# 123-code/Distributed-neural-networks

Measured on AMD Instinct MI355X. Metric: images/sec CIFAR-10 2-stage, higher is better.
Workload: dtype fp32 (bf16x3 split emulation, ~2^-16 per product); 1 GPU; model=cifar10-convnet (cifar_model_parts.py NeuralNetwork), global_batch=65536, parallelism=pp2-colocated, stages=2, microbatches=1, stage0_spare_cus=0, p2p=none, stage_cut=conv|fc (reference split, 16 KiB/img hop)

## Files before the change

### csrc/kernels/cifar_x3.hip

```cpp
#include <type_traits>

#include "gemm_epilogue.h"

namespace dnn {
namespace x3 {

template <bool PK>
__device__ __forceinline__ void split2(float a, float b, uint32_t& hi, uint32_t& lo) {
  if constexpr (PK) {
    hi = pack2bf_pk(a, b);
    const float ah = __uint_as_float(hi << 16), bh = __uint_as_float(hi & 0xffff0000u);
    float da = a - ah;
    const float db = b - bh;
    asm("" : "+v"(da));
    lo = pack2bf_pk(da, db);
  } else {
    hi = pack2bf(a, b);
    const float ah = __uint_as_float(hi << 16), bh = __uint_as_float(hi & 0xffff0000u);
    lo = pack2bf(a - ah, b - bh);
  }
}

__device__ __forceinline__ float4 buf_load16(const void* base, int bytes, int voff, int soff) {
#if defined(__HIP_DEVICE_COMPILE__)
  const auto rsrc = __builtin_amdgcn_make_buffer_rsrc(const_cast<void*>(base), 0, bytes, 0x00020000);
  return __builtin_bit_cast(float4, __builtin_amdgcn_raw_buffer_load_b128(rsrc, voff, soff, 0));
#else
  return float4{};
#endif
}
__device__ __forceinline__ void buf_glds16(const void* base, int bytes, int voff, int soff, void* lds_wave_base) {
#if defined(__HIP_DEVICE_COMPILE__)
  const auto rsrc = __builtin_amdgcn_make_buffer_rsrc(const_cast<void*>(base), 0, bytes, 0x00020000);
  __builtin_amdgcn_raw_ptr_buffer_load_lds(rsrc, (LDS_AS void*)lds_wave_base, 16, voff, soff, 0, 0);
#endif
}

__device__ __forceinline__ int dpp_xor1(int v) { return __builtin_amdgcn_mov_dpp(v, 0xB1, 0xF, 0xF, false); }
__device__ __forceinline__ int dpp_xor2(int v) { return __builtin_amdgcn_mov_dpp(v, 0x4E, 0xF, 0xF, false); }

constexpr int XW = 40;
constexpr int XPL = 34 * XW * 8;
constexpr int A1PL = 18 * 18 * 64;
constexpr int XP32 = 224;
constexpr int XPL32 = 34 * XP32;

template <int C1>
__device__ __forceinline__ constexpr int xpl() {
  return C1 ? XPL32 : XPL;
}
template <int C1>
__device__ __forceinline__ constexpr int lds_bytes() {
  return 4 * xpl<C1>() + 4 * A1PL;
}
constexpr int TAB_BYTES = 3 * 256 * 4;
struct U8Input {
  const unsigned char* x;
  const uint32_t* table;
};
template <int IN>
using s0_input_t = std::conditional_t<IN == 1, U8Input, const float* __restrict__>;

template <int C1>
__device__ __forceinline__ int xin_off(int k, int lo) {
  return ((k & 1) * 2 + lo) * xpl<C1>();
}
template <int C1>
__device__ __forceinline__ int a1_off(int k, int lo) {
  return 4 * xpl<C1>() + ((k & 1) * 2 + lo) * A1PL;
}

template <int S, int I, int LO>
__device__ __forceinline__ constexpr int c2_imm() {
  return (8 * I + (S >> 1) % 3) * 64 + LO * A1PL;
}

template <int S>
__device__ __forceinline__ void c2_issue(const uint32_t (&b)[3][2], bf16x8 (&a)[4]) {
  constexpr int ky = (S >> 1) / 3, par = S & 1;
  asm volatile("ds_read_b128 %0, %1 offset:%2" : "=v"(a[0]) : "v"(b[ky][par]), "i"(c2_imm<S, 0, 0>()));
  asm volatile("ds_read_b128 %0, %1 offset:%2" : "=v"(a[1]) : "v"(b[ky][par]), "i"(c2_imm<S, 1, 0>()));
  asm volatile("ds_read_b128 %0, %1 offset:%2" : "=v"(a[2]) : "v"(b[ky][par]), "i"(c2_imm<S, 0, 1>()));
  asm volatile("ds_read_b128 %0, %1 offset:%2" : "=v"(a[3]) : "v"(b[ky][par]), "i"(c2_imm<S, 1, 1>()));
}

template <int S>
__device__ __forceinline__ void c2_step(const uint32_t (&b)[3][2], const bf16x8 (&wh)[18], const bf16x8 (&wl)[18],
                                        f32x16 (&acc)[2], bf16x8 (&cur)[4], bf16x8 (&nxt)[4]) {
  if constexpr (S + 1 < 18) {
    c2_issue<S + 1>(b, nxt);
    asm volatile("s_waitcnt lgkmcnt(4)" ::: "memory");
  } else {
    asm volatile("s_waitcnt lgkmcnt(0)" ::: "memory");
  }
  __builtin_amdgcn_sched_barrier(0);
  acc[0] = __builtin_amdgcn_mfma_f32_32x32x16_bf16(cur[0], wh[S], acc[0], 0, 0, 0);
  acc[1] = __builtin_amdgcn_mfma_f32_32x32x16_bf16(cur[1], wh[S], acc[1], 0, 0, 0);
  acc[0] = __builtin_amdgcn_mfma_f32_32x32x16_bf16(cur[0], wl[S], acc[0], 0, 0, 0);
  acc[1] = __builtin_amdgcn_mfma_f32_32x32x16_bf16(cur[1], wl[S], acc[1], 0, 0, 0);
  acc[0] = __builtin_amdgcn_mfma_f32_32x32x16_bf16(cur[2], wh[S], acc[0], 0, 0, 0);
  acc[1] = __builtin_amdgcn_mfma_f32_32x32x16_bf16(cur[3], wh[S], acc[1], 0, 0, 0);
  __builtin_amdgcn_sched_barrier(0);
  if constexpr (S + 1 < 18) c2_step<S + 1>(b, wh, wl, acc, nxt, cur);
}

template <int N>
__device__ __forceinline__ void resident_fence(const bf16x8 (&w)[N]) {
#pragma unroll
  for (int i = 0; i < N; ++i) asm volatile("" ::"v"(w[i]));
}

template <int C2>
__device__ __forceinline__ int a1_swz(int Y) {
  return C2 ? (2 * Y) & 3 : Y & 3;
}

template <int T, int J, int LO>
__device__ __forceinline__ constexpr int m16_imm() {
  return (((T >> 1) / 3) * 18 + 4 * (2 * (T & 1) + J) + (T >> 1) % 3) * 64 + LO * A1PL;
}

template <int T>
__device__ __forceinline__ void m16_issue(const uint32_t (&b)[2], bf16x8 (&a)[4]) {
  constexpr int kyp = ((T >> 1) / 3) & 1;
  asm volatile("ds_read_b128 %0, %1 offset:%2" : "=v"(a[0]) : "v"(b[kyp]), "i"(m16_imm<T, 0, 0>()));
  asm volatile("ds_read_b128 %0, %1 offset:%2" : "=v"(a[1]) : "v"(b[kyp]), "i"(m16_imm<T, 1, 0>()));
  asm volatile("ds_read_b128 %0, %1 offset:%2" : "=v"(a[2]) : "v"(b[kyp]), "i"(m16_imm<T, 0, 1>()));
  asm volatile("ds_read_b128 %0, %1 offset:%2" : "=v"(a[3]) : "v"(b[kyp]), "i"(m16_imm<T, 1, 1>()));
}

template <int T>
__device__ __forceinline__ void m16_step(const uint32_t (&b)[2], const bf16x8 (&wh)[2][9], const bf16x8 (&wl)[2][9],
                                         f32x4 (&acc)[4][2], bf16x8 (&cur)[4], bf16x8 (&nxt)[4]) {
  constexpr int tap = T >> 1, m0 = 2 * (T & 1);
  if constexpr (T + 1 < 18) {
    m16_issue<T + 1>(b, nxt);
    asm volatile("s_waitcnt lgkmcnt(4)" ::: "memory");
  } else {
    asm volatile("s_waitcnt lgkmcnt(0)" ::: "memory");
  }
  __builtin_amdgcn_sched_barrier(0);
#pragma unroll
  for (int term = 0; term < 3; ++term)
#pragma unroll
    for (int nt = 0; nt < 2; ++nt)
#pragma unroll
      for (int j = 0; j < 2; ++j)
        acc[m0 + j][nt] = __builtin_amdgcn_mfma_f32_16x16x32_bf16(cur[(term == 2 ? 2 : 0) + j],
                                                                  term == 1 ? wl[nt][tap] : wh[nt][tap], acc[m0 + j][nt], 0, 0, 0);
  __builtin_amdgcn_sched_barrier(0);
  if constexpr (T + 1 < 18) m16_step<T + 1>(b, wh, wl, acc, nxt, cur);
}

template <bool SPLIT_OUT, int NT>
__device__ __forceinline__ void m16_epilogue(const f32x4 (&acc)[4][2], float bias, float* img, int oc, int PY, int x1) {
  float v[4];
#pragma unroll
  for (int mt = 0; mt < 4; ++mt) {
    const f32x4& a = acc[mt][NT];
    v[mt] = fmaxf(fmax_nan(fmax_nan(a[0], a[1]), fmax_nan(a[2], a[3])) + bias, 0.f);
  }
  const auto s0 = __builtin_amdgcn_permlane16_swap(__float_as_uint(v[0]), __float_as_uint(v[2]), false, false);
  const auto s1 = __builtin_amdgcn_permlane16_swap(__float_as_uint(v[1]), __float_as_uint(v[3]), false, false);
  if constexpr (SPLIT_OUT) {
    uint2 hi, lo;
    split2<true>(__uint_as_float(s0[0]), __uint_as_float(s0[1]), hi.x, lo.x);
    split2<true>(__uint_as_float(s1[0]), __uint_as_float(s1[1]), hi.y, lo.y);
    char* bp = reinterpret_cast<char*>(img) + (oc * 2 + (PY >> 2)) * 128 + ((PY & 3) * 8 + 4 * x1) * 2;
    *reinterpret_cast<uint2*>(bp) = hi;
    *reinterpret_cast<uint2*>(bp + 64) = lo;
  } else {
    *reinterpret_cast<uint4*>(img + oc * 64 + PY * 8 + 4 * x1) = make_uint4(s0[0], s0[1], s1[0], s1[1]);
  }
}

}

using namespace x3;

template <bool WIDE, bool SPLIT_OUT, int C2 = 0, int C1 = 0, int IN = 0>
__global__ __launch_bounds__(512, 1) void cifar_stage0_x3_kernel(
    s0_input_t<IN> x, float* __restrict__ out, const bf16_t* __restrict__ w1h,
    const bf16_t* __restrict__ w1l, const float* __restrict__ b1, const bf16_t* __restrict__ w2h,
    const bf16_t* __restrict__ w2l, const float* __restrict__ b2, int B) {
  static_assert(IN == 0 || C1 == 1, "uint8 input exists in the K = 32 producer only");
  constexpr int LDS_BYTES = lds_bytes<C1>();
  __shared__ __attribute__((aligned(16))) char smem[LDS_BYTES + (IN ? TAB_BYTES : 0)];
  const int tid = threadIdx.x, lane = tid & 63;
  const int wave = __builtin_amdgcn_readfirstlane(tid >> 6);
  const bool producer = wave < 4;
  const int rw = wave & 3;
  const int rt = tid & 255;
  const int h = lane >> 5, r32 = lane & 31;
  const int n = B > (int)blockIdx.x ? (B - 1 - (int)blockIdx.x) / (int)gridDim.x + 1 : 0;

  for (int i = tid; i < LDS_BYTES / 16; i += 512) reinterpret_cast<uint4*>(smem)[i] = make_uint4(0, 0, 0, 0);
  if constexpr (IN == 1)
    for (int i = tid; i < TAB_BYTES / 4; i += 512) reinterpret_cast<uint32_t*>(smem + LDS_BYTES)[i] = x.table[i];

  __syncthreads();

  if (producer) {
    const float bias = b1[r32];
    asm volatile("" ::"v"(bias));
    const int q = ((r32 & 1) ? 2 : 0) + ((r32 & 2) ? 1 : 0);
    const int cb = r32 & ~3;

    auto conv1_store = [&](const float (&v)[4], int Y0, int X0, int k) {
      const bool odd = r32 & 1;
      const int s0 = __float_as_int(odd ? v[0] : v[2]), s1 = __float_as_int(odd ? v[1] : v[3]);
      const float r0 = __int_as_float(dpp_xor1(s0)), r1 = __int_as_float(dpp_xor1(s1));
      uint32_t u0h, u0l, u1h, u1l;
      if (!odd) {
        split2<true>(v[0], r0, u0h, u0l);
        split2<true>(v[1], r1, u1h, u1l);
      } else {
        split2<true>(r0, v[2], u0h, u0l);
        split2<true>(r1, v[3], u1h, u1l);
      }
      const bool hi2 = r32 & 2;
      const uint32_t rch = (uint32_t)dpp_xor2((int)(hi2 ? u0h : u1h));
      const uint32_t rcl = (uint32_t)dpp_xor2((int)(hi2 ? u0l : u1l));
      const uint32_t mh = hi2 ? u1h : u0h, ml = hi2 ? u1l : u0l;
      uint2 wh, wl;
      wh.x = hi2 ? rch : mh;
      wh.y = hi2 ? mh : rch;
      wl.x = hi2 ? rcl : ml;
      wl.y = hi2 ? ml : rcl;
      const int Y = Y0 + (q >> 1), X = X0 + (q & 1);
      const int o = (Y * 18 + X) * 64 + ((((cb >> 3) ^ a1_swz<C2>(Y))) << 4) + (cb & 7) * 2;
      *reinterpret_cast<uint2*>(smem + a1_off<C1>(k, 0) + o) = wh;
      *reinterpret_cast<uint2*>(smem + a1_off<C1>(k, 1) + o) = wl;
    };
    auto produce = [&](auto&& load_img, auto&& stage_img, auto&& conv1_img) {
      if (n > 0) {
        load_img(0);
        stage_img(0);
        if (n > 1) load_img(1);
      }
      __syncthreads();
      for (int it = 0; it <= n; ++it) {
        if (it < n) {
          conv1_img(it);
          if (it + 1 < n) {
            stage_img(it + 1);
            if (it + 2 < n) load_img(it + 2);
          }
        }
        __syncthreads();
      }
    };

    if constexpr (C1 == 0 && IN == 0) {
      bf16x8 w1hf[3], w1lf[3];
#pragma unroll
      for (int s = 0; s < 3; ++s) {
        w1hf[s] = *reinterpret_cast<const bf16x8*>(w1h + r32 * 48 + s * 16 + h * 8);
        w1lf[s] = *reinterpret_cast<const bf16x8*>(w1l + r32 * 48 + s * 16 + h * 8);
      }
      resident_fence(w1hf);
      resident_fence(w1lf);

      float pf[4][3];
      auto load_img = [&](int k) {
        const float* xb = x + (size_t)(blockIdx.x + (size_t)k * gridDim.x) * 3072;
#pragma unroll
        for (int i = 0; i < 4; ++i)
#pragma unroll
          for (int c = 0; c < 3; ++c) pf[i][c] = xb[c * 1024 + rt + 256 * i];
      };
      auto stage_img = [&](int k) {
        char* xh = smem + xin_off<C1>(k, 0);
        char* xl = smem + xin_off<C1>(k, 1);
#pragma unroll
        for (int i = 0; i < 4; ++i) {
          const int p = rt + 256 * i, yy = p >> 5, xx = p & 31;
          uint2 vh, vl;
          split2<true>(pf[i][0], pf[i][1], vh.x, vl.x);
          split2<true>(pf[i][2], 0.f, vh.y, vl.y);
          const int o = ((yy + 1) * XW + xx + 1) * 8;
          *reinterpret_cast<uint2*>(xh + o) = vh;
          *reinterpret_cast<uint2*>(xl + o) = vl;
        }
      };
      const int c1_lane = ((r32 >> 3) * XW + (r32 & 7) + 2 * h) * 8;

      auto conv1_epi = [&](int t, const f32x16& acc, int k) {
        const int ty = t >> 2, tx = t & 3;
        float v[4];
#pragma unroll
        for (int qy = 0; qy < 2; ++qy)
#pragma unroll
          for (int qx = 0; qx < 2; ++qx) {
            const int g0 = (2 * qy) * 4 + 2 * qx;
            v[qy * 2 + qx] =
                fmaxf(fmax_nan(fmax_nan(acc[g0], acc[g0 + 1]), fmax_nan(acc[g0 + 4], acc[g0 + 5])) + bias, 0.f);
          }
        conv1_store(v, 2 * ty + 1, 4 * tx + 2 * h + 1, k);
      };
      auto frag = [&](const char* p) {
        const uint2 a = *reinterpret_cast<const uint2*>(p);
        const uint2 b = *reinterpret_cast<const uint2*>(p + 8);
        return __builtin_bit_cast(bf16x8, make_uint4(a.x, a.y, b.x, b.y));
      };
      auto conv1_pair = [&](int ta, int tb, int k) {
        const char* xh = smem + xin_off<C1>(k, 0);
        const int oa = c1_lane + ((4 * (ta >> 2)) * XW + 8 * (ta & 3)) * 8;
        const int ob = c1_lane + ((4 * (tb >> 2)) * XW + 8 * (tb & 3)) * 8;
        bf16x8 fah[3], fal[3], fbh[3], fbl[3];
#pragma unroll
        for (int s = 0; s < 3; ++s) {
          fah[s] = frag(xh + oa + s * XW * 8);
          fbh[s] = frag(xh + ob + s * XW * 8);
          fal[s] = frag(xh + XPL + oa + s * XW * 8);
          fbl[s] = frag(xh + XPL + ob + s * XW * 8);
        }
        f32x16 acca = {}, accb = {};
#pragma unroll
        for (int s = 0; s < 3; ++s) {
          acca = __builtin_amdgcn_mfma_f32_32x32x16_bf16(fah[s], w1hf[s], acca, 0, 0, 0);
          accb = __builtin_amdgcn_mfma_f32_32x32x16_bf16(fbh[s], w1hf[s], accb, 0, 0, 0);
          acca = __builtin_amdgcn_mfma_f32_32x32x16_bf16(fah[s], w1lf[s], acca, 0, 0, 0);
          accb = __builtin_amdgcn_mfma_f32_32x32x16_bf16(fbh[s], w1lf[s], accb, 0, 0, 0);
          acca = __builtin_amdgcn_mfma_f32_32x32x16_bf16(fal[s], w1hf[s], acca, 0, 0, 0);
          accb = __builtin_amdgcn_mfma_f32_32x32x16_bf16(fbl[s], w1hf[s], accb, 0, 0, 0);
        }
        conv1_epi(ta, acca, k);
        conv1_epi(tb, accb, k);
      };
      produce(load_img, stage_img, [&](int it) {
#pragma unroll 1
        for (int t = rw; t < 32; t += 8) conv1_pair(t, t + 4, it);
      });
    } else if constexpr (C1 == 1) {
      bf16x8 w1hf[2][2], w1lf[2][2];
#pragma unroll
      for (int par = 0; par < 2; ++par)
#pragma unroll
        for (int s = 0; s < 2; ++s) {
          w1hf[par][s] = *reinterpret_cast<const bf16x8*>(w1h + par * 1024 + r32 * 32 + s * 16 + h * 8);
          w1lf[par][s] = *reinterpret_cast<const bf16x8*>(w1l + par * 1024 + r32 * 32 + s * 16 + h * 8);
        }
      resident_fence(w1hf[0]);
      resident_fence(w1hf[1]);
      resident_fence(w1lf[0]);
      resident_fence(w1lf[1]);

      const int sj = rt & 7, r5 = rt >> 3;
      const int sy = (r5 & ~3) | ((r5 & 1) << 1) | ((r5 >> 1) & 1);
      std::conditional_t<IN == 1, uint32_t, float4> pf[3];
      auto load_img = [&](int k) {
        if constexpr (IN == 1) {
          const unsigned char* xb = x.x + (size_t)(blockIdx.x + (size_t)k * gridDim.x) * 3072 + sy * 96 + sj * 12;
#pragma unroll
          for (int c = 0; c < 3; ++c) pf[c] = *reinterpret_cast<const uint32_t*>(xb + 4 * c);
        } else {
          const float* xb = x + (size_t)(blockIdx.x + (size_t)k * gridDim.x) * 3072 + sy * 32 + sj * 4;
#pragma unroll
          for (int c = 0; c < 3; ++c) pf[c] = *reinterpret_cast<const float4*>(xb + c * 1024);
        }
      };
      auto stage_img = [&](int k) {
        const int o = (sy + 1) * XP32 + 8 + 24 * sj;
        char* xh = smem + xin_off<C1>(k, 0) + o;
        char* xl = smem + xin_off<C1>(k, 1) + o;
        uint2 vh[3], vl[3];
        if constexpr (IN == 1) {
          const char* tab = smem + LDS_BYTES;
          uint32_t e[12];
#pragma unroll
          for (int i = 0; i < 12; ++i)
            e[i] = *reinterpret_cast<const uint32_t*>(tab + (i % 3) * 1024 + ((pf[i >> 2] >> (8 * (i & 3))) & 0xffu) * 4);
          uint32_t ph[6], pl[6];
#pragma unroll
          for (int i = 0; i < 6; ++i) {
            ph[i] = __builtin_amdgcn_perm(e[2 * i + 1], e[2 * i], 0x05040100u);
            pl[i] = __builtin_amdgcn_perm(e[2 * i + 1], e[2 * i], 0x07060302u);
          }
#pragma unroll
          for (int i = 0; i < 3; ++i) {
            vh[i] = make_uint2(ph[2 * i], ph[2 * i + 1]);
            vl[i] = make_uint2(pl[2 * i], pl[2 * i + 1]);
          }
        } else {
          split2<true>(pf[0].x, pf[1].x, vh[0].x, vl[0].x);
          split2<true>(pf[2].x, pf[0].y, vh[0].y, vl[0].y);
          split2<true>(pf[1].y, pf[2].y, vh[1].x, vl[1].x);
          split2<true>(pf[0].z, pf[1].z, vh[1].y, vl[1].y);
          split2<true>(pf[2].z, pf[0].w, vh[2].x, vl[2].x);
          split2<true>(pf[1].w, pf[2].w, vh[2].y, vl[2].y);
        }
#pragma unroll
        for (int i = 0; i < 3; ++i) {
          *reinterpret_cast<uint2*>(xh + 8 * i) = vh[i];
          *reinterpret_cast<uint2*>(xl + 8 * i) = vl[i];
        }
      };
      const int rr = r32 >> 3, cc = r32 & 7;
      const int l0 = (rr + 2 * h) * XP32 + 12 * cc;
      int l1[4];
#pragma unroll
      for (int i = 0; i < 4; ++i)
        l1[i] = h ? (rr + (i < 2 ? i : 2)) * XP32 + 12 * cc + 16 : (rr + 1) * XP32 + 12 * cc + 4 * i;
      auto ld32 = [&](const char* p) { return *reinterpret_cast<const uint32_t*>(p); };
      auto conv1_pair = [&](int tp, int k) {
        const int ty = tp >> 1, tx2 = tp & 1;
        const char* xh = smem + xin_off<C1>(k, 0) + 4 * ty * XP32 + 96 * tx2;
        bf16x8 f[2][2][2];
#pragma unroll
        for (int par = 0; par < 2; ++par)
#pragma unroll
          for (int pl = 0; pl < 2; ++pl) {
            const char* p = xh + pl * XPL32 + 8 * par;
            f[par][pl][0] = __builtin_bit_cast(
                bf16x8, make_uint4(ld32(p + l0), ld32(p + l0 + 4), ld32(p + l0 + 8), ld32(p + l0 + 12)));
            f[par][pl][1] = __builtin_bit_cast(
                bf16x8, make_uint4(ld32(p + l1[0]), ld32(p + l1[1]), ld32(p + l1[2]), ld32(p + l1[3])));
          }
        f32x16 acca = {}, accb = {};
#pragma unroll
        for (int s = 0; s < 2; ++s) {
          acca = __builtin_amdgcn_mfma_f32_32x32x16_bf16(f[0][0][s], w1hf[0][s], acca, 0, 0, 0);
          accb = __builtin_amdgcn_mfma_f32_32x32x16_bf16(f[1][0][s], w1hf[1][s], accb, 0, 0, 0);
          acca = __builtin_amdgcn_mfma_f32_32x32x16_bf16(f[0][0][s], w1lf[0][s], acca, 0, 0, 0);
          accb = __builtin_amdgcn_mfma_f32_32x32x16_bf16(f[1][0][s], w1lf[1][s], accb, 0, 0, 0);
          acca = __builtin_amdgcn_mfma_f32_32x32x16_bf16(f[0][1][s], w1hf[0][s], acca, 0, 0, 0);
          accb = __builtin_amdgcn_mfma_f32_32x32x16_bf16(f[1][1][s], w1hf[1][s], accb, 0, 0, 0);
        }
#pragma unroll
        for (int e = 0; e < 2; ++e) {
          float v[4];
#pragma unroll
          for (int qy = 0; qy < 2; ++qy)
#pragma unroll
            for (int qx = 0; qx < 2; ++qx) {
              const int g = 8 * qy + 2 * e + qx;
              v[qy * 2 + qx] =
                  fmaxf(fmax_nan(fmax_nan(acca[g], accb[g]), fmax_nan(acca[g + 4], accb[g + 4])) + bias, 0.f);
            }
          conv1_store(v, 2 * ty + 1, 8 * tx2 + 4 * h + 2 * e + 1, k);
        }
      };
      produce(load_img, stage_img, [&](int it) {
#pragma unroll 1
        for (int tp = rw; tp < 16; tp += 4) conv1_pair(tp, it);
      });
    }
  } else if constexpr (C2 != 0) {
    const int m = lane & 15, q16 = lane >> 4, y1 = q16 >> 1, x1 = q16 & 1;
    const int oc = (rw & 1) * 32 + m;
    bf16x8 w2hf[2][9], w2lf[2][9];
#pragma unroll
    for (int nt = 0; nt < 2; ++nt)
#pragma unroll
      for (int tap = 0; tap < 9; ++tap) {
        w2hf[nt][tap] = *reinterpret_cast<const bf16x8*>(w2h + (oc + 16 * nt) * 288 + tap * 32 + q16 * 8);
        w2lf[nt][tap] = *reinterpret_cast<const bf16x8*>(w2l + (oc + 16 * nt) * 288 + tap * 32 + q16 * 8);
      }
    const float bias0 = b2[oc], bias1 = b2[oc + 16];
    resident_fence(w2hf[0]);
    resident_fence(w2hf[1]);
    resident_fence(w2lf[0]);
    resident_fence(w2lf[1]);
    asm volatile("" ::"v"(bias0), "v"(bias1));
    const int py = 2 * (m >> 3) + ((m >> 1) & 1), px = 2 * ((m >> 2) & 1) + (m & 1);
    uint32_t lb[2];
#pragma unroll
    for (int kyp = 0; kyp < 2; ++kyp) lb[kyp] = (uint32_t)((py * 18 + px) * 64 + ((q16 ^ a1_swz<C2>(py + kyp)) << 4));

    auto conv2_img = [&](int k) {
      float* img = out + (size_t)(blockIdx.x + (size_t)k * gridDim.x) * 4096;
      const uint32_t plane = (uint32_t)(uintptr_t)(smem + a1_off<C1>(k, 0));
#pragma unroll 1
      for (int p = 0; p < 2; ++p) {
        const int ty2 = (rw >> 1) * 2 + p;
        const uint32_t rb = plane + ty2 * 4 * 18 * 64;
        const uint32_t b[2] = {rb + lb[0], rb + lb[1]};
        f32x4 acc[4][2];
#pragma unroll
        for (int mt = 0; mt < 4; ++mt) acc[mt][0] = acc[mt][1] = f32x4{};
        bf16x8 a0[4], a1[4];
        m16_issue<0>(b, a0);
        m16_step<0>(b, w2hf, w2lf, acc, a0, a1);
        m16_epilogue<SPLIT_OUT, 0>(acc, bias0, img, oc, 2 * ty2 + y1, x1);
        m16_epilogue<SPLIT_OUT, 1>(acc, bias1, img, oc + 16, 2 * ty2 + y1, x1);
      }
    };

    __syncthreads();
    for (int it = 0; it <= n; ++it) {
      if (it >= 1) conv2_img(it - 1);
      __syncthreads();
    }
  } else {
    const int oc2 = (rw & 1) * 32 + r32;
    bf16x8 w2hf[18], w2lf[18];
#pragma unroll
    for (int s = 0; s < 18; ++s) {
      w2hf[s] = *reinterpret_cast<const bf16x8*>(w2h + oc2 * 288 + s * 16 + h * 8);
      w2lf[s] = *reinterpret_cast<const bf16x8*>(w2l + oc2 * 288 + s * 16 + h * 8);
    }
    const float bias = b2[oc2];
    resident_fence(w2hf);
    resident_fence(w2lf);
    asm volatile("" ::"v"(bias));
    uint32_t lb[3][2];
#pragma unroll
    for (int ky = 0; ky < 3; ++ky)
#pragma unroll
      for (int par = 0; par < 2; ++par) {
        const int yr = (r32 >> 3) + ky;
        lb[ky][par] = (uint32_t)((yr * 18 + (r32 & 7)) * 64 + (((2 * par + h) ^ (yr & 3)) << 4));
      }

    auto conv2_img = [&](int k) {
      float* ob = out + (size_t)(blockIdx.x + (size_t)k * gridDim.x) * 4096 + oc2 * 64;
      const uint32_t plane = (uint32_t)(uintptr_t)(smem + a1_off<C1>(k, 0));
#pragma unroll 1
      for (int p = 0; p < 2; ++p) {
        const int ty2 = (rw >> 1) * 2 + p;
        const uint32_t rb = plane + ty2 * 4 * 18 * 64;
        uint32_t b[3][2];
#pragma unroll
        for (int ky = 0; ky < 3; ++ky)
#pragma unroll
          for (int par = 0; par < 2; ++par) b[ky][par] = rb + lb[ky][par];
        f32x16 acc[2] = {f32x16{}, f32x16{}};
        bf16x8 a0[4], a1[4];
        c2_issue<0>(b, a0);
        c2_step<0>(b, w2hf, w2lf, acc, a0, a1);
        if constexpr (WIDE) {
#pragma unroll
          for (int qy = 0; qy < 2; ++qy) {
            const int g0 = (2 * qy) * 4;
            float v[2][2];
#pragma unroll
            for (int i = 0; i < 2; ++i) {
              v[i][0] = fmaxf(fmax_nan(fmax_nan(acc[i][g0], acc[i][g0 + 1]), fmax_nan(acc[i][g0 + 4], acc[i][g0 + 5])) + bias, 0.f);
              v[i][1] = fmaxf(fmax_nan(fmax_nan(acc[i][g0 + 2], acc[i][g0 + 3]), fmax_nan(acc[i][g0 + 6], acc[i][g0 + 7])) + bias,
                              0.f);
            }
            const auto sx = __builtin_amdgcn_permlane32_swap(__float_as_uint(v[0][0]), __float_as_uint(v[1][0]), false,
                                                             false);
            const auto sy = __builtin_amdgcn_permlane32_swap(__float_as_uint(v[0][1]), __float_as_uint(v[1][1]), false,
                                                             false);
            const int PY = 2 * ty2 + qy;
            if constexpr (SPLIT_OUT) {
              uint2 hi, lo;
              split2<true>(__uint_as_float(sx[0]), __uint_as_float(sy[0]), hi.x, lo.x);
              split2<true>(__uint_as_float(sx[1]), __uint_as_float(sy[1]), hi.y, lo.y);
              char* bp = reinterpret_cast<char*>(ob - oc2 * 64) + (oc2 * 2 + (PY >> 2)) * 128 + ((PY & 3) * 8 + 4 * h) * 2;
              *reinterpret_cast<uint2*>(bp) = hi;
              *reinterpret_cast<uint2*>(bp + 64) = lo;
            } else {
              *reinterpret_cast<uint4*>(ob + PY * 8 + 4 * h) = make_uint4(sx[0], sy[0], sx[1], sy[1]);
            }
          }
        } else {
#pragma unroll
        for (int i = 0; i < 2; ++i) {
#pragma unroll
          for (int qy = 0; qy < 2; ++qy) {
            float2 pv;
            const int g0 = (2 * qy) * 4;
            pv.x = fmaxf(fmax_nan(fmax_nan(acc[i][g0], acc[i][g0 + 1]), fmax_nan(acc[i][g0 + 4], acc[i][g0 + 5])) + bias, 0.f);
            pv.y = fmaxf(fmax_nan(fmax_nan(acc[i][g0 + 2], acc[i][g0 + 3]), fmax_nan(acc[i][g0 + 6], acc[i][g0 + 7])) + bias,
                         0.f);
            const int PY = 2 * ty2 + qy, PX = 4 * i + 2 * h;
            if constexpr (SPLIT_OUT) {
              uint32_t hi, lo;
              split2<true>(pv.x, pv.y, hi, lo);
              char* bp = reinterpret_cast<char*>(ob - oc2 * 64) + (oc2 * 2 + (PY >> 2)) * 128 + ((PY & 3) * 8 + PX) * 2;
              *reinterpret_cast<uint32_t*>(bp) = hi;
              *reinterpret_cast<uint32_t*>(bp + 64) = lo;
            } else {
              *reinterpret_cast<float2*>(ob + PY * 8 + PX) = pv;
            }
          }
        }
        }
      }
    };

    __syncthreads();
    for (int it = 0; it <= n; ++it) {
      if (it >= 1) conv2_img(it - 1);
      __syncthreads();
    }
  }
}

constexpr int F1_T = 256, F1_K = 32, F1_PLANE = 256 * 64;

__device__ __forceinline__ int f1_swz(int r) { return (r >> 2) & 2; }

__device__ __forceinline__ bf16x8 f1_frag(const char* plane, int row, int chunk) {
  return *reinterpret_cast<const bf16x8*>(plane + row * 64 + ((chunk ^ f1_swz(row)) << 4));
}

__device__ __forceinline__ void f1_tile_coords(int logical, int ntm, int ntn, int& tm, int& tn) {
  constexpr int G = 8;
  const int per = G * ntn, grp = logical / per, first = grp * G;
  const int gm = min(ntm - first, G), r = logical - grp * per;
  tm = first + r % gm;
  tn = r / gm;
}

template <bool SPLIT_IN, bool LEAN>
__global__ __launch_bounds__(512, 1) void cifar_fc1_x3_kernel(const float* __restrict__ A, int lda,
                                                              const bf16_t* __restrict__ Wh,
                                                              const bf16_t* __restrict__ Wl, int ldw,
                                                              const float* __restrict__ bias, float* __restrict__ C,
                                                              int ldc, int M, int N, int K) {
  __shared__ __attribute__((aligned(1024))) char smem[2 * 4 * F1_PLANE];
  const int tid = threadIdx.x, lane = tid & 63, wave = tid >> 6;
  const int ntn = N / F1_T, ntm = (M + F1_T - 1) / F1_T;
  int tm, tn;
  f1_tile_coords(xcd_remap(blockIdx.x, ntm * ntn), ntm, ntn, tm, tn);
  const int m0 = tm * F1_T, n0 = tn * F1_T;
  const int wr = wave >> 2, wc = wave & 3;
  const int nk = K / F1_K;
  auto plane = [&](int u, int p) { return smem + (u * 4 + p) * F1_PLANE; };

  int ltid = tid;
  float4 ar[4];
  const int wave_u = __builtin_amdgcn_readfirstlane(wave);
  int a_rows[4];
#pragma unroll
  for (int k = 0; k < 4; ++k) a_rows[k] = __builtin_amdgcn_readfirstlane(max(min(M - m0 - 64 * k, 64), 0));
  const float* const a_tile = A + (size_t)m0 * lda;
  const int a_tile_bytes = min(M - m0, F1_T) * lda * 4;
  auto dma_voff = [&](int ld_bytes) {
    return (wave * 32 + (lane >> 2)) * ld_bytes + (((lane & 3) ^ ((lane >> 4) & 2)) << 4);
  };
  int a_voff = 0, a_voff1 = 0, w_voff = 0;
  LDS_AS char* aw_base = nullptr;
  LDS_AS char* fa_base = nullptr;
  LDS_AS char* fw_base = nullptr;
  if constexpr (LEAN) {
    LDS_AS char* const lds = (LDS_AS char*)smem;
    const int fr = lane & 15, fc = lane >> 4;
    const int fo = fr * 64 + ((fc ^ ((fr >> 2) & 2)) << 4);
    fa_base = lds + (wave >> 2) * 128 * 64 + fo;
    fw_base = lds + 2 * F1_PLANE + (wave & 3) * 64 * 64 + fo;
    w_voff = dma_voff(ldw * 2);
    if constexpr (SPLIT_IN) {
      a_voff = dma_voff(lda * 4);
      a_voff1 = a_voff + 16 * lda * 4;
      asm volatile("" : "+v"(a_voff1));
    } else {
      const int r = tid >> 3, c = (tid & 7) >> 1, half = tid & 1;
      a_voff = r * lda * 4 + (tid & 7) * 16;
      aw_base = lds + r * 64 + ((c ^ f1_swz(r)) << 4) + half * 8;
      asm volatile("" : "+v"(aw_base));
    }
    asm volatile("" : "+v"(a_voff), "+v"(w_voff), "+v"(fa_base), "+v"(fw_base));
  }
  constexpr int F1_BUF = 4 * F1_PLANE;
  auto load_a = [&](int t, auto) {
    if constexpr (LEAN) {
#pragma unroll
      for (int k = 0; k < 4; ++k)
        ar[k] = buf_load16(A + (size_t)(m0 + 64 * k) * lda, a_rows[k] * lda * 4, a_voff, t * 128);
      return;
    }
    const int x = ltid;
#pragma unroll
    for (int k = 0; k < 4; ++k) {
      const int row = min(m0 + (x >> 3) + 64 * k, M - 1);
      ar[k] = *reinterpret_cast<const float4*>(A + (size_t)row * lda + t * F1_K + (x & 7) * 4);
    }
  };
  auto store_a = [&](int u, auto) {
    if constexpr (LEAN) {
      LDS_AS char* const w = aw_base + u * F1_BUF;
#pragma unroll
      for (int k = 0; k < 4; ++k) {
        uint2 hi, lo;
        split2<true>(ar[k].x, ar[k].y, hi.x, lo.x);
        split2<true>(ar[k].z, ar[k].w, hi.y, lo.y);
        typedef uint32_t u32x2 __attribute__((ext_vector_type(2)));
        *reinterpret_cast<LDS_AS u32x2*>(w + k * 4096) = u32x2{hi.x, hi.y};
        *reinterpret_cast<LDS_AS u32x2*>(w + F1_PLANE + k * 4096) = u32x2{lo.x, lo.y};
      }
      return;
    }
    const int x = ltid;
#pragma unroll
    for (int k = 0; k < 4; ++k) {
      const int r = (x >> 3) + 64 * k, c = (x & 7) >> 1, half = x & 1;
      uint2 hi, lo;
      split2<false>(ar[k].x, ar[k].y, hi.x, lo.x);
      split2<false>(ar[k].z, ar[k].w, hi.y, lo.y);
      const int o = r * 64 + ((c ^ f1_swz(r)) << 4) + half * 8;
      *reinterpret_cast<uint2*>(plane(u, 0) + o) = hi;
      *reinterpret_cast<uint2*>(plane(u, 1) + o) = lo;
    }
  };
  auto stage_a = [&](int u, int t) {
    if constexpr (LEAN) {
#pragma unroll
      for (int p = 0; p < 2; ++p)
#pragma unroll
        for (int j = 0; j < 2; ++j)
          buf_glds16(a_tile, a_tile_bytes, j ? a_voff1 : a_voff, t * 128 + p * 64,
                     plane(u, p) + (wave_u * 2 + j) * 1024);
      return;
    }
    const char* Ab = reinterpret_cast<const char*>(A);
    const int lane = ltid & 63, wave = ltid >> 6;
#pragma unroll
    for (int p = 0; p < 2; ++p) {
#pragma unroll
      for (int j = 0; j < 2; ++j) {
        const int piece = wave * 2 + j, rl = piece * 16 + (lane >> 2);
        const int c = (lane & 3) ^ f1_swz(rl);
        const int row = min(m0 + rl, M - 1);
        glds16(Ab + (size_t)row * lda * 4 + t * 128 + p * 64 + c * 16, plane(u, p) + piece * 1024);
      }
    }
  };
  auto stage_w = [&](int u, int t) {
    if constexpr (LEAN) {
#pragma unroll
      for (int p = 0; p < 2; ++p)
#pragma unroll
        for (int j = 0; j < 2; ++j)
          buf_glds16((p ? Wl : Wh) + (size_t)n0 * ldw, F1_T * ldw * 2, w_voff, j * 16 * ldw * 2 + t * 64,
                     plane(u, 2 + p) + (wave_u * 2 + j) * 1024);
      return;
    }
    const int lane = ltid & 63, wave = ltid >> 6;
#pragma unroll
    for (int p = 0; p < 2; ++p) {
      const bf16_t* W = p ? Wl : Wh;
#pragma unroll
      for (int j = 0; j < 2; ++j) {
        const int piece = wave * 2 + j, rl = piece * 16 + (lane >> 2);
        const int c = (lane & 3) ^ f1_swz(rl);
        glds16(W + (size_t)(n0 + rl) * ldw + t * F1_K + c * 8, plane(u, 2 + p) + piece * 1024);
      }
    }
  };

  f32x4 acc[8][4];
#pragma unroll
  for (int i = 0; i < 8; ++i)
#pragma unroll
    for (int j = 0; j < 4; ++j) acc[i][j] = f32x4{0.f, 0.f, 0.f, 0.f};

  using I0 = std::integral_constant<int, 0>;
  if constexpr (SPLIT_IN) {
    stage_a(0, 0);
    stage_w(0, 0);
    asm volatile("s_waitcnt vmcnt(0)" ::: "memory");
  } else {
    load_a(0, I0{});
    stage_w(0, 0);
    asm volatile("s_waitcnt vmcnt(0)" ::: "memory");
    store_a(0, I0{});
    if (nk > 1) load_a(1, I0{});
  }
  asm volatile("s_waitcnt lgkmcnt(0)" ::: "memory");
  __builtin_amdgcn_sched_barrier(0);
  __builtin_amdgcn_s_barrier();
  __builtin_amdgcn_sched_barrier(0);

  const int fr = lane & 15, fc = lane >> 4;
  auto barrier = [&]() {
    asm volatile("s_waitcnt lgkmcnt(0)" ::: "memory");
    __builtin_amdgcn_sched_barrier(0);
    __builtin_amdgcn_s_barrier();
    __builtin_amdgcn_sched_barrier(0);
  };
  bf16x8 fbh[4], fbl[4], fah[8], fal[8];
  auto read_frags = [&](int u) {
    if constexpr (LEAN) {
      LDS_AS char* const fw = fw_base + u * F1_BUF;
      LDS_AS char* const fa = fa_base + u * F1_BUF;
#pragma unroll
      for (int j = 0; j < 4; ++j) {
        fbh[j] = *reinterpret_cast<LDS_AS bf16x8*>(fw + j * 1024);
        fbl[j] = *reinterpret_cast<LDS_AS bf16x8*>(fw + F1_PLANE + j * 1024);
      }
#pragma unroll
      for (int i = 0; i < 8; ++i) {
        fah[i] = *reinterpret_cast<LDS_AS bf16x8*>(fa + i * 1024);
        fal[i] = *reinterpret_cast<LDS_AS bf16x8*>(fa + F1_PLANE + i * 1024);
      }
      return;
    }
    const int fr = ltid & 15, fc = (ltid >> 4) & 3, wc = (ltid >> 6) & 3, wr = ltid >> 8;
#pragma unroll
    for (int j = 0; j < 4; ++j) {
      fbh[j] = f1_frag(plane(u, 2), wc * 64 + j * 16 + fr, fc);
      fbl[j] = f1_frag(plane(u, 3), wc * 64 + j * 16 + fr, fc);
    }
#pragma unroll
    for (int i = 0; i < 8; ++i) {
      fah[i] = f1_frag(plane(u, 0), wr * 128 + i * 16 + fr, fc);
      fal[i] = f1_frag(plane(u, 1), wr * 128 + i * 16 + fr, fc);
    }
  };
  auto mfma_seg = [&]() {
    __builtin_amdgcn_sched_barrier(0);
#pragma unroll
    for (int i = 0; i < 8; ++i)
#pragma unroll
      for (int term = 0; term < 3; ++term)
#pragma unroll
        for (int j = 0; j < 4; ++j)
          acc[i][j] = __builtin_amdgcn_mfma_f32_16x16x32_bf16(term == 1 ? fbl[j] : fbh[j], term == 2 ? fal[i] : fah[i],
                                                              acc[i][j], 0, 0, 0);
    __builtin_amdgcn_sched_barrier(0);
  };
  auto retire_dma = [&](bool a_in_flight) {
    if (a_in_flight)
      asm volatile("s_waitcnt vmcnt(4)" ::: "memory");
    else
      asm volatile("s_waitcnt vmcnt(0)" ::: "memory");
  };
  auto stage_next = [&](int u, int t) {
    if constexpr (SPLIT_IN) stage_a(u, t);
    stage_w(u, t);
  };
  const bool g1 = __builtin_amdgcn_readfirstlane(wr) != 0;
  auto fresh_tid = [&]() {
    if constexpr (LEAN) return;
    ltid = tid;
    asm volatile("" : "+v"(ltid));
  };
// ... 348 lines not shown
```

Baseline: 31.84 million images/s.

## Raise conv2 wave priority early and use buffer loads/stores with precomputed lane offsets

```diff
diff --git a/csrc/kernels/cifar_x3.hip b/csrc/kernels/cifar_x3.hip
--- a/csrc/kernels/cifar_x3.hip
+++ b/csrc/kernels/cifar_x3.hip
@@ -29,6 +29,28 @@
   return float4{};
 #endif
 }
+__device__ __forceinline__ uint32_t buf_load4(const void* base, int bytes, int voff, int soff) {
+#if defined(__HIP_DEVICE_COMPILE__)
+  const auto rsrc = __builtin_amdgcn_make_buffer_rsrc(const_cast<void*>(base), 0, bytes, 0x00020000);
+  return __builtin_amdgcn_raw_buffer_load_b32(rsrc, voff, soff, 0);
+#else
+  return 0;
+#endif
+}
+__device__ __forceinline__ void buf_store16(void* base, int bytes, int voff, int soff, uint4 v) {
+#if defined(__HIP_DEVICE_COMPILE__)
+  typedef unsigned int u32x4 __attribute__((ext_vector_type(4)));
+  const auto rsrc = __builtin_amdgcn_make_buffer_rsrc(base, 0, bytes, 0x00020000);
+  __builtin_amdgcn_raw_buffer_store_b128(u32x4{v.x, v.y, v.z, v.w}, rsrc, voff, soff, 0);
+#endif
+}
+__device__ __forceinline__ void buf_store8(void* base, int bytes, int voff, int soff, uint2 v) {
+#if defined(__HIP_DEVICE_COMPILE__)
+  typedef unsigned int u32x2 __attribute__((ext_vector_type(2)));
+  const auto rsrc = __builtin_amdgcn_make_buffer_rsrc(base, 0, bytes, 0x00020000);
+  __builtin_amdgcn_raw_buffer_store_b64(u32x2{v.x, v.y}, rsrc, voff, soff, 0);
+#endif
+}
 __device__ __forceinline__ void buf_glds16(const void* base, int bytes, int voff, int soff, void* lds_wave_base) {
 #if defined(__HIP_DEVICE_COMPILE__)
   const auto rsrc = __builtin_amdgcn_make_buffer_rsrc(const_cast<void*>(base), 0, bytes, 0x00020000);
@@ -44,6 +66,7 @@
 constexpr int A1PL = 18 * 18 * 64;
 constexpr int XP32 = 224;
 constexpr int XPL32 = 34 * XP32;
+constexpr int C2_PRIO_STEPS = 9;
 
 template <int C1>
 __device__ __forceinline__ constexpr int xpl() {
@@ -87,6 +110,7 @@
 template <int S>
 __device__ __forceinline__ void c2_step(const uint32_t (&b)[3][2], const bf16x8 (&wh)[18], const bf16x8 (&wl)[18],
                                         f32x16 (&acc)[2], bf16x8 (&cur)[4], bf16x8 (&nxt)[4]) {
+  if constexpr (S == C2_PRIO_STEPS) __builtin_amdgcn_s_setprio(0);
   if constexpr (S + 1 < 18) {
     c2_issue<S + 1>(b, nxt);
     asm volatile("s_waitcnt lgkmcnt(4)" ::: "memory");
@@ -133,6 +157,7 @@
 __device__ __forceinline__ void m16_step(const uint32_t (&b)[2], const bf16x8 (&wh)[2][9], const bf16x8 (&wl)[2][9],
                                          f32x4 (&acc)[4][2], bf16x8 (&cur)[4], bf16x8 (&nxt)[4]) {
   constexpr int tap = T >> 1, m0 = 2 * (T & 1);
+  if constexpr (T == C2_PRIO_STEPS) __builtin_amdgcn_s_setprio(0);
   if constexpr (T + 1 < 18) {
     m16_issue<T + 1>(b, nxt);
     asm volatile("s_waitcnt lgkmcnt(4)" ::: "memory");
@@ -153,7 +178,7 @@
 }
 
 template <bool SPLIT_OUT, int NT>
-__device__ __forceinline__ void m16_epilogue(const f32x4 (&acc)[4][2], float bias, float* img, int oc, int PY, int x1) {
+__device__ __forceinline__ void m16_epilogue(const f32x4 (&acc)[4][2], float bias, float* img, int lane, int p) {
   float v[4];
 #pragma unroll
   for (int mt = 0; mt < 4; ++mt) {
@@ -166,11 +191,10 @@
     uint2 hi, lo;
     split2<true>(__uint_as_float(s0[0]), __uint_as_float(s0[1]), hi.x, lo.x);
     split2<true>(__uint_as_float(s1[0]), __uint_as_float(s1[1]), hi.y, lo.y);
-    char* bp = reinterpret_cast<char*>(img) + (oc * 2 + (PY >> 2)) * 128 + ((PY & 3) * 8 + 4 * x1) * 2;
-    *reinterpret_cast<uint2*>(bp) = hi;
-    *reinterpret_cast<uint2*>(bp + 64) = lo;
+    buf_store8(img, 16384, lane, 32 * p + 4096 * NT, hi);
+    buf_store8(img, 16384, lane, 32 * p + 4096 * NT + 64, lo);
   } else {
-    *reinterpret_cast<uint4*>(img + oc * 64 + PY * 8 + 4 * x1) = make_uint4(s0[0], s0[1], s1[0], s1[1]);
+    buf_store16(img, 16384, lane, 64 * p + 4096 * NT, make_uint4(s0[0], s0[1], s1[0], s1[1]));
   }
 }
 
@@ -206,18 +230,18 @@
     const int q = ((r32 & 1) ? 2 : 0) + ((r32 & 2) ? 1 : 0);
     const int cb = r32 & ~3;
 
-    auto conv1_store = [&](const float (&v)[4], int Y0, int X0, int k) {
+    auto a1_lane = [&](int par, int xh) {
+      const int Y = 2 * par + 1 + (q >> 1);
+      return ((q >> 1) * 18 + (q & 1) + xh) * 64 + ((((cb >> 3) ^ a1_swz<C2>(Y))) << 4) + (cb & 7) * 2;
+    };
+    auto conv1_store = [&](const float (&v)[4], int ob) {
       const bool odd = r32 & 1;
       const int s0 = __float_as_int(odd ? v[0] : v[2]), s1 = __float_as_int(odd ? v[1] : v[3]);
       const float r0 = __int_as_float(dpp_xor1(s0)), r1 = __int_as_float(dpp_xor1(s1));
       uint32_t u0h, u0l, u1h, u1l;
-      if (!odd) {
-        split2<true>(v[0], r0, u0h, u0l);
-        split2<true>(v[1], r1, u1h, u1l);
-      } else {
-        split2<true>(r0, v[2], u0h, u0l);
-        split2<true>(r1, v[3], u1h, u1l);
-      }
+      const float k0 = odd ? v[2] : v[0], k1 = odd ? v[3] : v[1];
+      split2<true>(odd ? r0 : k0, odd ? k0 : r0, u0h, u0l);
+      split2<true>(odd ? r1 : k1, odd ? k1 : r1, u1h, u1l);
       const bool hi2 = r32 & 2;
       const uint32_t rch = (uint32_t)dpp_xor2((int)(hi2 ? u0h : u1h));
       const uint32_t rcl = (uint32_t)dpp_xor2((int)(hi2 ? u0l : u1l));
@@ -227,10 +251,8 @@
       wh.y = hi2 ? mh : rch;
       wl.x = hi2 ? rcl : ml;
       wl.y = hi2 ? ml : rcl;
-      const int Y = Y0 + (q >> 1), X = X0 + (q & 1);
-      const int o = (Y * 18 + X) * 64 + ((((cb >> 3) ^ a1_swz<C2>(Y))) << 4) + (cb & 7) * 2;
-      *reinterpret_cast<uint2*>(smem + a1_off<C1>(k, 0) + o) = wh;
-      *reinterpret_cast<uint2*>(smem + a1_off<C1>(k, 1) + o) = wl;
+      *reinterpret_cast<uint2*>(smem + ob) = wh;
+      *reinterpret_cast<uint2*>(smem + ob + A1PL) = wl;
     };
     auto produce = [&](auto&& load_img, auto&& stage_img, auto&& conv1_img) {
       if (n > 0) {
@@ -267,7 +289,8 @@
 #pragma unroll
         for (int i = 0; i < 4; ++i)
 #pragma unroll
-          for (int c = 0; c < 3; ++c) pf[i][c] = xb[c * 1024 + rt + 256 * i];
+          for (int c = 0; c < 3; ++c)
+            pf[i][c] = __uint_as_float(buf_load4(xb, 12288, 4 * rt, 4 * (c * 1024 + 256 * i)));
       };
       auto stage_img = [&](int k) {
         char* xh = smem + xin_off<C1>(k, 0);
@@ -285,7 +308,8 @@
       };
       const int c1_lane = ((r32 >> 3) * XW + (r32 & 7) + 2 * h) * 8;
 
-      auto conv1_epi = [&](int t, const f32x16& acc, int k) {
+      const int a1l[2] = {a1_lane(0, 2 * h), a1_lane(1, 2 * h)};
+      auto conv1_epi = [&](int t, const f32x16& acc, int k, int par) {
         const int ty = t >> 2, tx = t & 3;
         float v[4];
 #pragma unroll
@@ -296,7 +320,7 @@
             v[qy * 2 + qx] =
                 fmaxf(fmax_nan(fmax_nan(acc[g0], acc[g0 + 1]), fmax_nan(acc[g0 + 4], acc[g0 + 5])) + bias, 0.f);
           }
-        conv1_store(v, 2 * ty + 1, 4 * tx + 2 * h + 1, k);
+        conv1_store(v, a1l[par] + a1_off<C1>(k, 0) + ((2 * ty + 1) * 18 + 4 * tx + 1) * 64);
       };
       auto frag = [&](const char* p) {
         const uint2 a = *reinterpret_cast<const uint2*>(p);
@@ -325,8 +349,8 @@
           acca = __builtin_amdgcn_mfma_f32_32x32x16_bf16(fal[s], w1hf[s], acca, 0, 0, 0);
           accb = __builtin_amdgcn_mfma_f32_32x32x16_bf16(fbl[s], w1hf[s], accb, 0, 0, 0);
         }
-        conv1_epi(ta, acca, k);
-        conv1_epi(tb, accb, k);
+        conv1_epi(ta, acca, k, 0);
+        conv1_epi(tb, accb, k, 1);
       };
       produce(load_img, stage_img, [&](int it) {
 #pragma unroll 1
@@ -349,15 +373,16 @@
       const int sj = rt & 7, r5 = rt >> 3;
       const int sy = (r5 & ~3) | ((r5 & 1) << 1) | ((r5 >> 1) & 1);
       std::conditional_t<IN == 1, uint32_t, float4> pf[3];
+      const int ld_lane = IN == 1 ? sy * 96 + sj * 12 : (sy * 32 + sj * 4) * 4;
       auto load_img = [&](int k) {
         if constexpr (IN == 1) {
-          const unsigned char* xb = x.x + (size_t)(blockIdx.x + (size_t)k * gridDim.x) * 3072 + sy * 96 + sj * 12;
-#pragma unroll
-          for (int c = 0; c < 3; ++c) pf[c] = *reinterpret_cast<const uint32_t*>(xb + 4 * c);
+          const unsigned char* xb = x.x + (size_t)(blockIdx.x + (size_t)k * gridDim.x) * 3072;
+#pragma unroll
+          for (int c = 0; c < 3; ++c) pf[c] = buf_load4(xb, 3072, ld_lane, 4 * c);
         } else {
-          const float* xb = x + (size_t)(blockIdx.x + (size_t)k * gridDim.x) * 3072 + sy * 32 + sj * 4;
-#pragma unroll
-          for (int c = 0; c < 3; ++c) pf[c] = *reinterpret_cast<const float4*>(xb + c * 1024);
+          const float* xb = x + (size_t)(blockIdx.x + (size_t)k * gridDim.x) * 3072;
+#pragma unroll
+          for (int c = 0; c < 3; ++c) pf[c] = buf_load16(xb, 12288, ld_lane, c * 4096);
         }
       };
       auto stage_img = [&](int k) {
@@ -403,6 +428,7 @@
       for (int i = 0; i < 4; ++i)
         l1[i] = h ? (rr + (i < 2 ? i : 2)) * XP32 + 12 * cc + 16 : (rr + 1) * XP32 + 12 * cc + 4 * i;
       auto ld32 = [&](const char* p) { return *reinterpret_cast<const uint32_t*>(p); };
+      const int a1l = a1_lane((rw >> 1) & 1, 4 * h);
       auto conv1_pair = [&](int tp, int k) {
         const int ty = tp >> 1, tx2 = tp & 1;
         const char* xh = smem + xin_off<C1>(k, 0) + 4 * ty * XP32 + 96 * tx2;
@@ -438,7 +464,7 @@
               v[qy * 2 + qx] =
                   fmaxf(fmax_nan(fmax_nan(acca[g], accb[g]), fmax_nan(acca[g + 4], accb[g + 4])) + bias, 0.f);
             }
-          conv1_store(v, 2 * ty + 1, 8 * tx2 + 4 * h + 2 * e + 1, k);
+          conv1_store(v, a1l + a1_off<C1>(k, 0) + ((2 * ty + 1) * 18 + 8 * tx2 + 2 * e + 1) * 64);
         }
       };
       produce(load_img, stage_img, [&](int it) {
@@ -468,6 +494,8 @@
 #pragma unroll
     for (int kyp = 0; kyp < 2; ++kyp) lb[kyp] = (uint32_t)((py * 18 + px) * 64 + ((q16 ^ a1_swz<C2>(py + kyp)) << 4));
 
+    const int st_lane = SPLIT_OUT ? (oc * 2 + (rw >> 1)) * 128 + (y1 * 8 + 4 * x1) * 2
+                                  : (oc * 64 + ((rw >> 1) * 4 + y1) * 8 + 4 * x1) * 4;
     auto conv2_img = [&](int k) {
       float* img = out + (size_t)(blockIdx.x + (size_t)k * gridDim.x) * 4096;
       const uint32_t plane = (uint32_t)(uintptr_t)(smem + a1_off<C1>(k, 0));
@@ -480,10 +508,11 @@
 #pragma unroll
         for (int mt = 0; mt < 4; ++mt) acc[mt][0] = acc[mt][1] = f32x4{};
         bf16x8 a0[4], a1[4];
+        __builtin_amdgcn_s_setprio(1);
         m16_issue<0>(b, a0);
         m16_step<0>(b, w2hf, w2lf, acc, a0, a1);
-        m16_epilogue<SPLIT_OUT, 0>(acc, bias0, img, oc, 2 * ty2 + y1, x1);
-        m16_epilogue<SPLIT_OUT, 1>(acc, bias1, img, oc + 16, 2 * ty2 + y1, x1);
+        m16_epilogue<SPLIT_OUT, 0>(acc, bias0, img, st_lane, p);
+        m16_epilogue<SPLIT_OUT, 1>(acc, bias1, img, st_lane, p);
       }
     };
 
@@ -527,6 +556,7 @@
           for (int par = 0; par < 2; ++par) b[ky][par] = rb + lb[ky][par];
         f32x16 acc[2] = {f32x16{}, f32x16{}};
         bf16x8 a0[4], a1[4];
+        __builtin_amdgcn_s_setprio(1);
         c2_issue<0>(b, a0);
         c2_step<0>(b, w2hf, w2lf, acc, a0, a1);
         if constexpr (WIDE) {
```

Measured after the change: 32.45 million images/s (median of 6 runs). 1.02x the previous value.
